# AbbVie-ComputationalGenomics/SAIGEgds

Measured on AMD Instinct MI355X. Metric: variants/sec seqAssocGLMM_SPA at N=430K; achieved HBM GB/s vs roofline, higher is better.
Workload: dtype f64

## Files before the change

saigegds_amd/csrc/kern_score3.h:

```cpp
#pragma once
#include <type_traits>

#ifndef S3_V4I_DEFINED
#define S3_V4I_DEFINED
typedef int s3_v4i __attribute__((ext_vector_type(4)));
#endif

#include "s3_layout.h"

template <int OFF> __device__ __forceinline__ void s3_ds_read(s3_v4i &dst, uint32_t addr)
{
	asm volatile("ds_read_b128 %0, %1 offset:%2" : "=v"(dst) : "v"(addr), "n"(OFF));
}
template <int N> __device__ __forceinline__ void s3_lgkm_wait(s3_v4i &reg) { asm volatile("s_waitcnt lgkmcnt(%1)" : "+v"(reg) : "n"(N)); }
__device__ __forceinline__ void s3_tie(s3_v4i &reg) { asm volatile("" : "+v"(reg)); }
#define S3_DS_READ(dst, addr, off) s3_ds_read<(off)>(dst, addr)
#define S3_LGKM_WAIT(n, reg) s3_lgkm_wait<(n)>(reg)
#define S3_TIE(reg) s3_tie(reg)

template <int I, int N, typename F>
__device__ __forceinline__ void s3_static_for(F &&f)
{
	if constexpr (I < N) { f(std::integral_constant<int, I>()); s3_static_for<I + 1, N>(f); }
}

#ifndef S3_AUX_ROWS
#define S3_AUX_ROWS 2
#endif
#define S3_WAITCNT_VM(n) __builtin_amdgcn_s_waitcnt(((n) & 0xF) | (((n) >> 4) << 14) | (0x7 << 4) | (0xF << 8))

template <int OP>
__device__ __forceinline__ void s3_unpack_op(uint32_t w, uint32_t &w4, s3_v4i &val, s3_v4i &b1)
{
	if constexpr (OP == 0) w4 = w >> 4;
	else if constexpr (OP == 1) val[0] = (int)(w & 0x03030303u);
	else if constexpr (OP == 2) val[1] = (int)(w & 0x0C0C0C0Cu);
	else if constexpr (OP == 3) val[2] = (int)(w4 & 0x03030303u);
	else if constexpr (OP == 4) val[3] = (int)(w4 & 0x0C0C0C0Cu);
	else if constexpr (OP == 5) b1[0] = (int)(w & 0x02020202u);
	else if constexpr (OP == 6) b1[1] = (int)(w & 0x08080808u);
	else if constexpr (OP == 7) b1[2] = (int)(w4 & 0x02020202u);
	else if constexpr (OP == 8) b1[3] = (int)(w4 & 0x08080808u);
}
#define S3_UNPACK3_OPS 15
template <int OP>
__device__ __forceinline__ void s3_unpack3_op(uint32_t w, uint32_t &w4, uint32_t &t, uint32_t &t4, s3_v4i &val, s3_v4i &b1, s3_v4i &mis)
{
	if constexpr (OP < 9) s3_unpack_op<OP>(w, w4, val, b1);
	else if constexpr (OP == 9) t = w >> 1;
	else if constexpr (OP == 10) t4 = w4 >> 1;
	else if constexpr (OP == 11) mis[0] = (int)(w & t & 0x01010101u);
	else if constexpr (OP == 12) mis[1] = (int)(w & t & 0x04040404u);
	else if constexpr (OP == 13) mis[2] = (int)(w4 & t4 & 0x01010101u);
	else if constexpr (OP == 14) mis[3] = (int)(w4 & t4 & 0x04040404u);
}

template <int NBF, int NAF, int NC, int NLA, int NLB, int DA, int DB, int ABL = 0, int NCB = 1, int NBUF_ = 2, int RM = 0, bool MISS = false>
__global__ void __launch_bounds__(64 * (NC + NLA + NLB), (NC + NLA + NLB + 3) / 4)
score3_kernel(const uint8_t *__restrict__ A, const uint8_t *__restrict__ Fl, S3Plan pl, int *__restrict__ out, unsigned long long *__restrict__ stamps)
{
#if __HIP_DEVICE_COMPILE__
	static_assert(NC % NCB == 0 && NCB >= 1 && NCB <= 4, "consumer waves = variant groups x column groups");
	constexpr int NCV = NC / NCB;
	constexpr int NBWMAX = (NBF + NCB - 1) / NCB;
	constexpr int NCOL = 16 * NBF;
	constexpr int TILE_BYTES = 16 * NCOL * 16;
	constexpr int NPB = TILE_BYTES / 1024;
	constexpr int NPA = NCV * NAF;
	constexpr int RA = DA + 1, RB = DB + 1;
	constexpr int SLOT_A = (RM == 1 ? 2 : 1) * NPA * 1024;
	static_assert(DA >= 1 && DB >= 1, "at least one tile ahead");
	extern __shared__ __attribute__((aligned(16))) uint8_t s3_smem[];

	const int tid = threadIdx.x, lane = tid & 63, wid = tid >> 6;
	const int x = blockIdx.x & 7, y = blockIdx.x >> 3;
	const int g = x % pl.ng, i = y * (8 / pl.ng) + x / pl.ng;
	const int nk = pl.rf + (i < pl.rem * pl.f ? 1 : 0);
	const int T0 = 2 * (int)((long long)g * (pl.ntile / 2) / pl.ng), T1 = 2 * (int)((long long)(g + 1) * (pl.ntile / 2) / pl.ng);
	unsigned long long st0 = 0, sr0 = 0;
	if (ABL & 16) { st0 = __builtin_amdgcn_s_memtime(); sr0 = __builtin_amdgcn_s_memrealtime(); }

	struct Pos { int k, t, t1, vtile, id; };
	auto pos_set = [&](Pos &p, int k) {
		p.k = k;
		if (k >= nk) return;
		if (k < pl.rf) { p.vtile = k * pl.wpg + i; p.t = T0; p.t1 = T1; p.id = g * pl.ipg + p.vtile; }
		else {
			const int q = i % pl.f, vv = i / pl.f, len = T1 - T0;
			p.vtile = pl.rf * pl.wpg + vv;
			p.t = T0 + 2 * (q * (len / 2) / pl.f); p.t1 = T0 + 2 * ((q + 1) * (len / 2) / pl.f);
			p.id = g * pl.ipg + pl.rf * pl.wpg + i;
		}
	};
	auto pos_next = [&](Pos &p) { if (++p.t >= p.t1) pos_set(p, p.k + 1); };
	Pos pc;
	pos_set(pc, 0);

	if (wid >= NC) {
		const bool rows = wid < NC + NLA;
		const int l = __builtin_amdgcn_readfirstlane(rows ? wid - NC : wid - NC - NLA);
		const int voff = (rows ? s3_dma_lane(lane) : lane) * 16;
		const unsigned rm_bpv = (unsigned)pl.bpv;
		Pos pa = pc;
		int sl = 0;
		int ahead = 0;
		if (rows && RM == 1) {
			constexpr int PLO = NPA / NLA, NHI = NPA % NLA;
			static_assert(2 * (PLO + 1) * (DA > 1 ? DA - 1 : 1) < 64, "vmcnt range");
			const int li = lane >> 3, lj = lane & 7;
			const int rlast = pl.nrow - 1 - 16 * (pl.nfrag - 1);
			unsigned vo[2], vol[2];
#pragma unroll
			for (int h = 0; h < 2; h++) {
				const unsigned c = (unsigned)(lj ^ ((li >> 1) | (h << 2)));
				vo[h] = (unsigned)(8 * h + li) * rm_bpv + c * 16u;
				vol[h] = (unsigned)min(8 * h + li, rlast) * rm_bpv + c * 16u;
			}
			auto issue = [&]() {
				const size_t f0 = (size_t)pa.vtile * pl.fpw;
				const __amdgpu_buffer_rsrc_t rsA = __builtin_amdgcn_make_buffer_rsrc((void *)(A + f0 * 16 * (size_t)pl.bpv), 0, 0xFFFFFFFFu, 0x00020000);
				const int lastf = pl.nfrag - 1 - (int)f0;
#pragma unroll
				for (int j = 0; j <= PLO; j++) {
					const int p = l + j * NLA;
					if (p >= NPA || (ABL & 2)) break;
					const int pp = min(p, lastf);
					const int so = (int)((unsigned)pp * 16u * rm_bpv + (unsigned)(pa.t >> 1) * 128u);
#pragma unroll
					for (int h = 0; h < 2; h++)
						__builtin_amdgcn_raw_ptr_buffer_load_lds(rsA, (__attribute__((address_space(3))) void *)(s3_smem + RB * TILE_BYTES + sl * SLOT_A + (2 * p + h) * 1024),
							16, (int)(pp == lastf ? vol[h] : vo[h]), so, 0, S3_AUX_ROWS);
				}
				sl = sl + 1 == RA ? 0 : sl + 1;
				pos_next(pa); pos_next(pa);
			};
#pragma unroll
			for (int d = 0; d < DA; d++) if (pa.k < nk) { issue(); ahead++; }
			while (pc.k < nk) {
				if (ahead == DA && DA > 1) { if (l < NHI) S3_WAITCNT_VM(2 * (PLO + 1) * (DA - 1)); else S3_WAITCNT_VM(2 * PLO * (DA - 1)); }
				else S3_WAITCNT_VM(0);
				__builtin_amdgcn_s_barrier();
				ahead--;
				if (pa.k < nk) { issue(); ahead++; }
				pos_next(pc);
				__builtin_amdgcn_s_barrier();
				pos_next(pc);
			}
		} else if (rows) {
			constexpr int PLO = NPA / NLA, NHI = NPA % NLA;
			static_assert((PLO + 1) * (DA - 1) < 64, "vmcnt range");
			auto issue = [&]() {
				const size_t f0 = (size_t)pa.vtile * pl.fpw;
				const __amdgpu_buffer_rsrc_t rsA = __builtin_amdgcn_make_buffer_rsrc(
					(void *)(A + (RM ? f0 * 16 * (size_t)pl.bpv : f0 * pl.ntile * 1024)), 0, 0xFFFFFFFFu, 0x00020000);
				const int lastf = pl.nfrag - 1 - (int)f0;
#pragma unroll
				for (int j = 0; j <= PLO; j++) {
					const int p = l + j * NLA;
					if (p >= NPA || (ABL & 2)) break;
					if constexpr (RM == 1) {
					} else if constexpr (RM == 2) {
						const int pp = min(p, lastf);
						__builtin_amdgcn_raw_ptr_buffer_load_lds(rsA, (__attribute__((address_space(3))) void *)(s3_smem + RB * TILE_BYTES + sl * SLOT_A + p * 1024),
							16, (int)((unsigned)(lane >> 3) * rm_bpv + (unsigned)(lane & 7) * 16u),
							(int)(((unsigned)pp * 16u + (unsigned)(pa.t & 1) * 8u) * rm_bpv + (unsigned)(pa.t >> 1) * 128u), 0, 0);
					} else
					__builtin_amdgcn_raw_ptr_buffer_load_lds(rsA, (__attribute__((address_space(3))) void *)(s3_smem + RB * TILE_BYTES + sl * SLOT_A + p * 1024),
						16, voff, (min(p, lastf) * pl.ntile + pa.t) * 1024, 0, 0);
				}
				sl = sl + 1 == RA ? 0 : sl + 1;
				pos_next(pa);
			};
#pragma unroll
			for (int d = 0; d < DA; d++) if (pa.k < nk) { issue(); ahead++; }
			while (pc.k < nk) {
				if (ahead == DA && DA > 1) { if (l < NHI) S3_WAITCNT_VM((PLO + 1) * (DA - 1)); else S3_WAITCNT_VM(PLO * (DA - 1)); }
				else S3_WAITCNT_VM(0);
				__builtin_amdgcn_s_barrier();
				ahead--;
				if (pa.k < nk) { issue(); ahead++; }
				pos_next(pc);
			}
		} else {
			constexpr int PLO = NPB / NLB, NHI = NPB % NLB;
			static_assert((PLO + 1) * (DB - 1) < 64, "vmcnt range");
			const __amdgpu_buffer_rsrc_t rsB = __builtin_amdgcn_make_buffer_rsrc((void *)Fl, 0, 0xFFFFFFFFu, 0x00020000);
			auto issue = [&]() {
#pragma unroll
				for (int j = 0; j <= PLO; j++) {
					const int b = l + j * NLB;
					if (b >= NPB || (ABL & 4)) break;
					__builtin_amdgcn_raw_ptr_buffer_load_lds(rsB, (__attribute__((address_space(3))) void *)(s3_smem + sl * TILE_BYTES + b * 1024),
						16, voff, pa.t * TILE_BYTES + b * 1024, 0, 0);
				}
				sl = sl + 1 == RB ? 0 : sl + 1;
				pos_next(pa);
			};
#pragma unroll
			for (int d = 0; d < DB; d++) if (pa.k < nk) { issue(); ahead++; }
			while (pc.k < nk) {
				if (ahead == DB && DB > 1) { if (l < NHI) S3_WAITCNT_VM((PLO + 1) * (DB - 1)); else S3_WAITCNT_VM(PLO * (DB - 1)); }
				else S3_WAITCNT_VM(0);
				__builtin_amdgcn_s_barrier();
				ahead--;
				if (pa.k < nk) { issue(); ahead++; }
				pos_next(pc);
			}
		}
		return;
	}

	const int r = lane & 15, kg = lane >> 4;
	const int vg = __builtin_amdgcn_readfirstlane(wid / NCB), cgr = __builtin_amdgcn_readfirstlane(wid % NCB);
	const uint32_t smem_lds = (uint32_t)(uintptr_t)(__attribute__((address_space(3))) uint8_t *)s3_smem;
	const uint32_t ring_lds = smem_lds + RB * TILE_BYTES + vg * (NAF * 1024) + lane * 16;
	const int rm_sig = ((r & 7) >> 1) | ((r >> 3) << 2);
	const uint32_t ring_rm = smem_lds + RB * TILE_BYTES + vg * (NAF * 2048) + (uint32_t)(r >> 3) * 1024u + (uint32_t)(r & 7) * 128u;
	const uint32_t ring_rm0 = ring_rm + (uint32_t)(kg ^ rm_sig) * 16u, ring_rm1 = ring_rm + (uint32_t)((4 + kg) ^ rm_sig) * 16u;

	auto consume = [&](auto CG) {
		constexpr int cg = decltype(CG)::value;
		constexpr int B0 = cg * NBWMAX;
		constexpr int NBW = (NBF - B0 < NBWMAX) ? NBF - B0 : NBWMAX;
		constexpr bool HASB1 = B0 + NBW == NBF;
		static_assert(NBW >= 1, "empty column group");
		const uint32_t bt_lds = smem_lds + (4 * kg * NCOL + r) * 16 + B0 * 256;

		s3_v4i acc[NAF][NBW];
#pragma unroll
		for (int f = 0; f < NAF; f++)
#pragma unroll
			for (int b = 0; b < NBW; b++) acc[f][b] = (s3_v4i){0, 0, 0, 0};

		constexpr int BCH = NBUF_ > 2 ? 1 : NCB > 1 ? (NBW <= 2 ? NBW : 2) : (NBF <= 4 ? NBF : (NBF >= 9 ? 2 : (NBF % 3 == 0 ? 3 : 4)));
		constexpr int NBUF = NBUF_;
		constexpr bool PIPE = NCB == 1 && NBF <= 8;
		constexpr int NCH = (NBW + BCH - 1) / BCH;
		constexpr int NM = NAF * NBW;
		constexpr int NV = HASB1 ? 4 * NAF : 0, NW = 5 * NAF;
		constexpr int BLV = HASB1 ? NBW - 2 : NBW - 1;
		constexpr int MB = HASB1 ? ((!PIPE && NBW >= 3) ? (NBW - 2) * NAF : (NBW - 1) * NAF) : 0;
		static_assert(!HASB1 || NBW >= 2 || NCB == 1, "a column group of the b1 fragment alone has no slot for its unpack");

		int sa = 0, sb = 0;
		int par = 0;
		while (pc.k < nk) {
			__builtin_amdgcn_sched_barrier(0);
			__builtin_amdgcn_s_barrier();
			__builtin_amdgcn_sched_barrier(0);
			const uint32_t a_addr = (RM == 1 ? (par ? ring_rm1 : ring_rm0) : ring_lds) + (uint32_t)(sa * SLOT_A);
			constexpr int AFS = RM == 1 ? 2048 : 1024;
			const uint32_t b_addr = bt_lds + (uint32_t)(sb * TILE_BYTES);
			s3_v4i aw[NAF];
			s3_static_for<0, NAF>([&](auto F) { constexpr int f = decltype(F)::value; S3_DS_READ(aw[f], a_addr, f * AFS); });
			s3_v4i bf[NBUF][BCH];
			auto read_chunk = [&](auto CI) {
				constexpr int ci = decltype(CI)::value, u = ci / NCH, b0 = (ci % NCH) * BCH;
				s3_static_for<0, BCH>([&](auto J) {
					constexpr int j = decltype(J)::value;
					if constexpr (b0 + j < NBW) {
						if (ABL & 8) bf[ci % NBUF][j] = (s3_v4i){u, j, r, sa};
						else S3_DS_READ(bf[ci % NBUF][j], b_addr, u * NCOL * 16 + (b0 + j) * 256);
					}
				});
			};
			constexpr int nread_last = NBW - (NCH - 1) * BCH;
			auto nreads = [](int c0, int c1) constexpr { int n = 0; for (int c = c0; c < c1 && c < 4 * NCH; c++) n += (c % NCH == NCH - 1) ? nread_last : BCH; return n; };
			s3_static_for<0, NBUF - 1>([&](auto C) { if constexpr (decltype(C)::value < 4 * NCH) read_chunk(C); });
			if (!(ABL & 8)) { S3_LGKM_WAIT(nreads(0, NBUF - 1), aw[0]); } else { S3_LGKM_WAIT(0, aw[0]); }
#pragma unroll
			for (int f = 1; f < NAF; f++) S3_TIE(aw[f]);
			s3_v4i val[PIPE ? 2 : 1][NAF], b1[NAF];
			uint32_t w4[PIPE ? 2 : 1][NAF];
			if (!(ABL & 1)) {
				s3_static_for<0, (PIPE ? NW : 5)>([&](auto O) {
					constexpr int o = decltype(O)::value, f = o / 5, op = o % 5;
					s3_unpack_op<op>((uint32_t)aw[f][0], w4[0][f], val[0][f], b1[f]);
				});
			}
			__builtin_amdgcn_sched_barrier(0);
			constexpr bool FM = !PIPE && BCH == 2 && nread_last == 2;
			constexpr int M0 = (NCH - 1) * BCH * NAF;
			s3_static_for<0, 4>([&](auto U) {
				constexpr int u = decltype(U)::value;
				constexpr int vb = PIPE ? (u & 1) : 0, vn = PIPE ? ((u + 1) & 1) : 0;
				s3_static_for<0, NM>([&](auto MI) {
					constexpr int m = decltype(MI)::value;
					constexpr bool fm = FM && m >= M0;
					constexpr int b = fm ? (NCH - 1) * BCH + (m - M0) % 2 : m / NAF, f = fm ? (m - M0) / 2 : m % NAF;
					constexpr int ch = b / BCH, ci = u * NCH + ch, j = b % BCH;
					if constexpr (m == ch * BCH * NAF) {
						if constexpr (ci + NBUF - 1 < 4 * NCH) read_chunk(std::integral_constant<int, ci + NBUF - 1>());
						constexpr int inflight = (ABL & 8) ? 0 : nreads(ci + 1, ci + NBUF);
						constexpr int nb = (ch == NCH - 1) ? nread_last : BCH;
						S3_LGKM_WAIT(inflight, bf[ci % NBUF][0]);
#pragma unroll
						for (int jj = 1; jj < nb; jj++) S3_TIE(bf[ci % NBUF][jj]);
					}
					if (ABL & 1) { if (f == 0) acc[0][b][1] ^= bf[ci % NBUF][j][0] ^ aw[b % NAF][u]; }
					else if (HASB1 && b == NBW - 1) acc[f][b] = __builtin_amdgcn_mfma_i32_16x16x64_i8(b1[f], bf[ci % NBUF][j], acc[f][b], 0, 0, 0);
					else acc[f][b] = __builtin_amdgcn_mfma_i32_16x16x64_i8(val[vb][f], bf[ci % NBUF][j], acc[f][b], 0, 0, 0);
					if (!(ABL & 1)) {
						if constexpr (!PIPE && u == 0 && b == 0 && f + 1 < NAF) {
							s3_static_for<0, 5>([&](auto O) {
								constexpr int op = decltype(O)::value;
								s3_unpack_op<op>((uint32_t)aw[f + 1][0], w4[0][f + 1], val[0][f + 1], b1[f + 1]);
							});
						}
						if constexpr (m < MB) {
							s3_static_for<m * NV / MB, (m + 1) * NV / MB>([&](auto O) {
								constexpr int o = decltype(O)::value, ff = o / 4, op = 5 + o % 4;
								s3_unpack_op<op>((uint32_t)aw[ff][u], w4[vb][ff], val[vb][ff], b1[ff]);
							});
						}
						if constexpr (PIPE && u < 3) {
							s3_static_for<m * NW / NM, (m + 1) * NW / NM>([&](auto O) {
								constexpr int o = decltype(O)::value, ff = o / 5, op = o % 5;
								s3_unpack_op<op>((uint32_t)aw[ff][u + 1], w4[vn][ff], val[vn][ff], b1[ff]);
							});
						}
						if constexpr (!PIPE && u < 3) {
							constexpr int lo = !fm ? ((b == BLV || (BLV < 0 && b == 0)) ? 0 : 5) : (HASB1 ? (j == 0 ? 0 : 2) : (j == 1 ? 0 : 5));
							constexpr int hi = !fm ? 5 : (HASB1 && j == 0 ? 2 : 5);
							s3_static_for<lo, hi>([&](auto O) {
								constexpr int op = decltype(O)::value;
								s3_unpack_op<op>((uint32_t)aw[f][u + 1], w4[0][f], val[0][f], b1[f]);
							});
						}
					}
					__builtin_amdgcn_sched_barrier(0);
				});
			});
			if (pc.t + 1 == pc.t1) {
				int *dst = out + ((size_t)pc.id * NC + wid) * (NAF * NBWMAX * 256) + lane;
#pragma unroll
				for (int f = 0; f < NAF; f++)
#pragma unroll
					for (int b = 0; b < NBW; b++)
#pragma unroll
						for (int reg = 0; reg < 4; reg++) {
							dst[((f * NBWMAX + b) * 4 + reg) * 64] = acc[f][b][reg];
							acc[f][b][reg] = 0;
						}
			}
			pos_next(pc);
			if (RM != 1 || par) sa = sa + 1 == RA ? 0 : sa + 1;
			sb = sb + 1 == RB ? 0 : sb + 1;
			par ^= 1;
		}
	};
	auto consume3 = [&]() {
		static_assert(!MISS || NCB == 1, "the three-plane form has one column group");
		constexpr int NBUF = NBUF_;
		constexpr int NBV = NBF - 1;
		constexpr int NVF = 2 * NBV + 1;
		constexpr int NM = NAF * NVF;
		constexpr int NOPT = S3_UNPACK3_OPS * NAF;
		constexpr int BCH = NBF <= 4 ? NBF : 2, NCH = (NBF + BCH - 1) / BCH;
		const uint32_t bt_lds = smem_lds + (4 * kg * NCOL + r) * 16;
		s3_v4i acc[NAF][NBF], accm[NAF][NBV > 0 ? NBV : 1];
#pragma unroll
		for (int f = 0; f < NAF; f++) {
#pragma unroll
			for (int b = 0; b < NBF; b++) acc[f][b] = (s3_v4i){0, 0, 0, 0};
#pragma unroll
			for (int b = 0; b < NBV; b++) accm[f][b] = (s3_v4i){0, 0, 0, 0};
		}
		int sa = 0, sb = 0, par = 0;
		while (pc.k < nk) {
			__builtin_amdgcn_sched_barrier(0);
			__builtin_amdgcn_s_barrier();
			__builtin_amdgcn_sched_barrier(0);
			const uint32_t a_addr = (RM == 1 ? (par ? ring_rm1 : ring_rm0) : ring_lds) + (uint32_t)(sa * SLOT_A);
			constexpr int AFS = RM == 1 ? 2048 : 1024;
			const uint32_t b_addr = bt_lds + (uint32_t)(sb * TILE_BYTES);
			s3_v4i aw[NAF];
			s3_static_for<0, NAF>([&](auto F) { constexpr int f = decltype(F)::value; S3_DS_READ(aw[f], a_addr, f * AFS); });
			s3_v4i bf[NBUF][BCH];
			auto read_chunk = [&](auto CI) {
				constexpr int ci = decltype(CI)::value, u = ci / NCH, b0 = (ci % NCH) * BCH;
				s3_static_for<0, BCH>([&](auto J) {
					constexpr int j = decltype(J)::value;
					if constexpr (b0 + j < NBF) S3_DS_READ(bf[ci % NBUF][j], b_addr, u * NCOL * 16 + (b0 + j) * 256);
				});
			};
			constexpr int nread_last = NBF - (NCH - 1) * BCH;
			auto nreads = [](int c0, int c1) constexpr { int n = 0; for (int c = c0; c < c1 && c < 4 * NCH; c++) n += (c % NCH == NCH - 1) ? nread_last : BCH; return n; };
			s3_static_for<0, NBUF - 1>([&](auto C) { if constexpr (decltype(C)::value < 4 * NCH) read_chunk(C); });
			S3_LGKM_WAIT(nreads(0, NBUF - 1), aw[0]);
#pragma unroll
			for (int f = 1; f < NAF; f++) S3_TIE(aw[f]);
			s3_v4i val[2][NAF], b1[2][NAF], mis[2][NAF];
			uint32_t w4[NAF], tt[NAF], m4[NAF];
			s3_static_for<0, NOPT>([&](auto O) {
				constexpr int o = decltype(O)::value, f = o / S3_UNPACK3_OPS, op = o % S3_UNPACK3_OPS;
				s3_unpack3_op<op>((uint32_t)aw[f][0], w4[f], tt[f], m4[f], val[0][f], b1[0][f], mis[0][f]);
			});
			__builtin_amdgcn_sched_barrier(0);
			s3_static_for<0, 4>([&](auto U) {
				constexpr int u = decltype(U)::value, vb = u & 1, vn = (u + 1) & 1;
				s3_static_for<0, NM>([&](auto MI) {
					constexpr int m = decltype(MI)::value, vf = m / NAF, f = m % NAF;
					constexpr int b = vf < 2 * NBV ? vf / 2 : NBV;
					constexpr int plane = vf < 2 * NBV ? (vf & 1) : 2;
					constexpr int ch = b / BCH, ci = u * NCH + ch, j = b % BCH;
					if constexpr (f == 0 && plane != 1 && b % BCH == 0) {
						if constexpr (ci + NBUF - 1 < 4 * NCH) read_chunk(std::integral_constant<int, ci + NBUF - 1>());
						constexpr int inflight = nreads(ci + 1, ci + NBUF);
						constexpr int nb = (ch == NCH - 1) ? nread_last : BCH;
						S3_LGKM_WAIT(inflight, bf[ci % NBUF][0]);
#pragma unroll
						for (int jj = 1; jj < nb; jj++) S3_TIE(bf[ci % NBUF][jj]);
					}
					if constexpr (plane == 0) acc[f][b] = __builtin_amdgcn_mfma_i32_16x16x64_i8(val[vb][f], bf[ci % NBUF][j], acc[f][b], 0, 0, 0);
					else if constexpr (plane == 1) accm[f][b] = __builtin_amdgcn_mfma_i32_16x16x64_i8(mis[vb][f], bf[ci % NBUF][j], accm[f][b], 0, 0, 0);
					else acc[f][b] = __builtin_amdgcn_mfma_i32_16x16x64_i8(b1[vb][f], bf[ci % NBUF][j], acc[f][b], 0, 0, 0);
					if constexpr (u < 3) {
						s3_static_for<m * NOPT / NM, (m + 1) * NOPT / NM>([&](auto O) {
							constexpr int o = decltype(O)::value, ff = o / S3_UNPACK3_OPS, op = o % S3_UNPACK3_OPS;
							s3_unpack3_op<op>((uint32_t)aw[ff][u + 1], w4[ff], tt[ff], m4[ff], val[vn][ff], b1[vn][ff], mis[vn][ff]);
						});
					}
					__builtin_amdgcn_sched_barrier(0);
				});
			});
			if (pc.t + 1 == pc.t1) {
				int *dst = out + ((size_t)pc.id * NC + wid) * (NAF * NVF * 256) + lane;
#pragma unroll
				for (int f = 0; f < NAF; f++) {
#pragma unroll
					for (int b = 0; b < NBF; b++)
#pragma unroll
						for (int reg = 0; reg < 4; reg++) { dst[((f * NVF + b) * 4 + reg) * 64] = acc[f][b][reg]; acc[f][b][reg] = 0; }
#pragma unroll
					for (int b = 0; b < NBV; b++)
#pragma unroll
						for (int reg = 0; reg < 4; reg++) { dst[((f * NVF + NBF + b) * 4 + reg) * 64] = accm[f][b][reg]; accm[f][b][reg] = 0; }
				}
			}
			pos_next(pc);
			if (RM != 1 || par) sa = sa + 1 == RA ? 0 : sa + 1;
			sb = sb + 1 == RB ? 0 : sb + 1;
			par ^= 1;
		}
	};
	if constexpr (MISS) consume3();
	else if constexpr (NCB == 1) consume(std::integral_constant<int, 0>());
	else s3_static_for<0, NCB>([&](auto CG) { if (cgr == decltype(CG)::value) consume(CG); });
	if ((ABL & 16) && tid == 0) {
		stamps[2 * blockIdx.x] = __builtin_amdgcn_s_memtime() - st0;
		stamps[2 * blockIdx.x + 1] = __builtin_amdgcn_s_memrealtime() - sr0;
	}
#endif
}

#define S3_FOR_EACH_NBF(X) \
	X(2, 4, 8, 3, 1, 1, 2) X(3, 4, 8, 3, 1, 1, 1) X(4, 4, 8, 3, 1, 1, 1) X(5, 3, 8, 3, 1, 1, 2) X(6, 3, 8, 3, 1, 1, 1) \
	X(7, 4, 4, 2, 2, 2, 1) X(8, 4, 4, 2, 2, 2, 1) X(9, 4, 4, 2, 2, 1, 1) X(10, 4, 4, 2, 2, 1, 1) X(11, 4, 4, 2, 2, 1, 1) \
	X(12, 3, 4, 2, 2, 1, 1) X(13, 3, 4, 2, 2, 1, 1) X(14, 2, 4, 2, 2, 2, 1) X(15, 2, 4, 2, 2, 1, 1) X(16, 2, 4, 2, 2, 1, 1)
#define S3_FOR_EACH_NBF_MISS(X) \
	X(2, 4, 8, 3, 1, 1, 2) X(3, 3, 8, 3, 1, 1, 2) X(4, 2, 8, 3, 1, 2, 2) X(5, 2, 8, 3, 1, 2, 2) X(6, 3, 4, 2, 2, 2, 1) \
	X(7, 2, 4, 2, 2, 2, 1) X(8, 2, 4, 2, 2, 2, 1) X(9, 2, 4, 2, 2, 2, 1) X(10, 2, 4, 2, 2, 2, 1) X(11, 1, 4, 2, 2, 2, 1) \
	X(12, 1, 4, 2, 2, 2, 1) X(13, 1, 4, 2, 2, 2, 1) X(14, 1, 4, 2, 2, 2, 1) X(15, 1, 4, 2, 2, 2, 1) X(16, 1, 4, 2, 2, 2, 1)
static inline size_t s3_lds_bytes(int NBF, int NAF, int NC, int DA, int DB) { return ((size_t)(DB + 1) * 4 * NBF + (size_t)(DA + 1) * 2 * NC * NAF) * 1024; }

#ifndef S3_KERNEL_ONLY
#include "kern_lists.h"

__device__ __forceinline__ unsigned long long s3_block_excl(unsigned long long x, unsigned long long *sh)
{
	const int tid = threadIdx.x;
	sh[tid] = x;
	__syncthreads();
	for (int o = 1; o < 1024; o <<= 1) {
		const unsigned long long y = tid >= o ? sh[tid - o] : 0;
		__syncthreads();
		sh[tid] += y;
		__syncthreads();
	}
	const unsigned long long incl = sh[tid];
	__syncthreads();
	return incl - x;
}

__global__ void __launch_bounds__(256)
s3_ingest_clist_count_kernel(int M, int N, int lim, int *__restrict__ nzv ,
	const int *__restrict__ n2v, const int *__restrict__ n3, uint8_t *__restrict__ corient)
{
	const int v = blockIdx.x * 256 + threadIdx.x;
	if (v >= M) return;
	const int nz = nzv[v], n2 = n2v[v], m3 = n3[v];
	const long long AC = (long long)(nz - n2 - m3) + 2ll * n2;
	const bool minus = (double)AC / (2.0 * (double)(N - m3)) > 0.5;
	const int nnz = minus ? N - n2 : nz;
	const int orient = (N - m3 > 0 && nnz <= lim) ? (minus ? 2 : 1) : 0;
	corient[v] = (uint8_t)orient;
	nzv[v] = orient ? nnz : 0;
}

__global__ void __launch_bounds__(1024)
s3_ingest_clist_kernel(int M, unsigned cidx_cap, const int *__restrict__ cn, unsigned *__restrict__ cptr, uint8_t *__restrict__ corient)
{
	__shared__ unsigned long long sh[1024];
	const int tid = threadIdx.x, per = (M + 1023) / 1024, v0 = tid * per, v1 = min(M, v0 + per);
	unsigned long long mine = 0;
	for (int v = v0; v < v1; v++) mine += (unsigned long long)cn[v];
	unsigned long long base = s3_block_excl(mine, sh);
	for (int v = v0; v < v1; v++) {
		const int n = cn[v];
		const bool fits = base + (unsigned long long)n <= (unsigned long long)cidx_cap;
		cptr[v] = (unsigned)min(base, (unsigned long long)cidx_cap);
		if (!fits) corient[v] = 0;
		else base += (unsigned long long)n;
	}
	if (tid == 1023) cptr[M] = (unsigned)min(base, (unsigned long long)cidx_cap);
}

template <int PP>
__global__ void __launch_bounds__(256, PP <= 16 ? 8 : 7)
s3_t3_kernel(int M, int P, const long long *__restrict__ Q, S3Lists L, long long *__restrict__ part)
{
	constexpr int TPW = 64 / PP;
	constexpr int NB = 1;
	const int lane = threadIdx.x & 63, wid = threadIdx.x >> 6;
	const int g = blockIdx.x % L.nr, chunk = blockIdx.x / L.nr;
	const unsigned *__restrict__ idx = L.idx;
	const int c = lane % PP, tk = lane / PP;
	const int v = (chunk * 4 + wid) * TPW + tk;
	unsigned e0 = 0, e1 = 0;
	if (v < M) { e0 = L.lstart[(size_t)g * L.ld + v]; e1 = e0 + (unsigned)max(0, L.lcnt[(size_t)g * L.ld + v]); }
	long long hi = 0, lo = 0;
	const int gbase = lane - c;
	for (unsigned e = e0; __any(e < e1); e += NB * PP) {
		unsigned mine[NB];
#pragma unroll
		for (int k = 0; k < NB; k++) mine[k] = (e + k * PP + c < e1) ? idx[e + k * PP + c] : 0xFFFFFFFFu;
		constexpr int UN = PP <= 16 ? 8 : 4;
		constexpr int UNR = PP <= 16 ? 2 : 1;
#pragma unroll
		for (int k = 0; k < NB; k++)
#pragma unroll UNR
			for (int j0 = 0; j0 < PP; j0 += UN) {
				long long q[UN];
#pragma unroll
				for (int j = 0; j < UN; j++) {
					const unsigned s = (unsigned)__shfl((int)mine[k], gbase + j0 + j, 64);
					q[j] = (s != 0xFFFFFFFFu && c < P) ? Q[(size_t)s * P + c] : 0;
				}
#pragma unroll
				for (int j = 0; j < UN; j++) { hi += q[j] >> 32; lo += q[j] & 0xFFFFFFFFll; }
			}
	}
	if (v < M && c < P) {
		long long *o = part + (((size_t)g * M + v) * P + c) * 2;
		o[0] = hi; o[1] = lo;
	}
}

__global__ void __launch_bounds__(256)
s3_reduce_kernel(S3Plan pl, int M, int NCW, int NAF, int NBF, int NCB, const int *__restrict__ slabs, int *__restrict__ accbuf, int stride,
	int *__restrict__ counters, int *__restrict__ cursors)
{
	if (blockIdx.x == 0 && blockIdx.y == 0 && threadIdx.x < 32) {
		if (threadIdx.x < 24) counters[threadIdx.x] = 0;
		if (threadIdx.x < 8 && cursors) cursors[threadIdx.x] = 0;
	}
	const int NBW = (NBF + NCB - 1) / NCB;
	const int e = (blockIdx.x * 256 + threadIdx.x) * 4, per = NCW * NAF * NBW * 256, vtile = blockIdx.y;
	if (e >= per) return;
	const int lane = e & 63, reg = (e >> 6) & 3, fb = e >> 8;
	const int bw = fb % NBW, wf = fb / NBW;
	const int wave = wf / NAF, f = wf - wave * NAF;
	const int b = (wave % NCB) * NBW + bw;
	if (b >= NBF) return;
	const int v = (vtile * pl.fpw + (wave / NCB) * NAF + f) * 16 + (lane >> 4) * 4 + reg;
	if (v >= M) return;
	s3_v4i sum = (s3_v4i){0, 0, 0, 0};
	for (int g = 0; g < pl.ng; g++) {
		int first, count;
		s3_items_of(pl, vtile, g, first, count);
		for (int id = first; id < first + count; id++) sum += *reinterpret_cast<const s3_v4i *>(slabs + (size_t)id * per + e);
	}
	*reinterpret_cast<s3_v4i *>(accbuf + (size_t)v * stride + b * 16 + (lane & 15)) = sum;
}

__host__ __device__ constexpr int s3e_vb(int K) { return K <= 8 ? 256 : 128; }
template <int K>
__global__ void __launch_bounds__(256)
score3_epilogue(int M, DevModel md, MfEpi ep, const int *__restrict__ accbuf, int acc_stride, int miss_off,
	const long long *__restrict__ t3part , int nr,
	const int *__restrict__ lcnt , size_t ld, int *__restrict__ ovf_list,
	SpaRec *__restrict__ recs, int *__restrict__ counters, int btop, int *__restrict__ fb_series, int *__restrict__ fb_exact,
	double *__restrict__ out8, uint8_t *__restrict__ valid, double guard_tol, int dbg = 0)
{
	constexpr int P = 2 * K + 2, CW = P - 1;
	constexpr int S3E_VB = s3e_vb(K);
	__shared__ double s_acc[S3E_VB][P | 1];
	__shared__ double s_imp[S3E_VB];
	__shared__ int s_n[S3E_VB][4];
	__shared__ long long s_ftot[P][2];
	__shared__ int s_col[P][3];
	const int tid = threadIdx.x, j0 = blockIdx.x * S3E_VB;
	const int N = md.N;
	if (dbg & 1) {
		if (tid == 0)
#pragma unroll
			for (int c = 0; c < P; c++) {
				s_col[c][0] = ep.ccol[c]; s_col[c][1] = ep.climb[c]; s_col[c][2] = ep.escale[c];
				s_ftot[c][0] = ep.ftot_hi[c]; s_ftot[c][1] = ep.ftot_lo[c];
			}
	} else
	for (int c = tid; c < P; c += S3E_VB) {
		s_col[c][0] = ep.ccol[c]; s_col[c][1] = ep.climb[c]; s_col[c][2] = ep.escale[c];
		s_ftot[c][0] = ep.ftot_hi[c]; s_ftot[c][1] = ep.ftot_lo[c];
	}
	{
		const int j = j0 + tid;
		const int *a0 = accbuf + (size_t)min(j, M - 1) * acc_stride;
		int n3 = 0;
		bool over = false;
		if (miss_off) n3 = a0[miss_off + ep.col_ones] / 4;
		else {
			for (int g0 = 0; g0 < nr; g0 += 8) {
				int cn[8];
#pragma unroll
				for (int u = 0; u < 8; u++) cn[u] = lcnt[(size_t)min(g0 + u, nr - 1) * ld + min(j, M - 1)];
#pragma unroll
				for (int u = 0; u < 8; u++) if (g0 + u < nr) { over |= cn[u] < 0; n3 += cn[u] < 0 ? 0 : cn[u]; }
			}
		}
		if (j >= M) n3 = 0;
		{
			const int tot = wave_total_i(n3);
			if ((tid & 63) == 0 && tot >= 64) atomicAdd(&counters[22], tot >> 6);
		}
		int state = 0, n1 = 0, n2 = 0;
		double imp = 0;
		if (dbg & 8) over = false;
		if (j < M) {
			if (over) ovf_list[atomicAdd(&counters[23], 1)] = j;
			else {
				const long long AC = (long long)(a0[ep.col_ones] / 4) - 3ll * n3;
				n2 = a0[ep.col_b1 + ep.climb[CW]] / 8 - n3;
				n1 = (int)(AC - 2ll * n2);
				const VarHead h = make_head(md, (double)AC, N - n3);
				if (!h.pass) { nan_row(out8 + (size_t)j * 8); valid[j] = 0; }
				else { state = h.minus ? 2 : 1; imp = 2 * h.AF; }
			}
		}
		s_n[tid][0] = n1; s_n[tid][1] = n2; s_n[tid][2] = n3; s_n[tid][3] = state;
		s_imp[tid] = imp;
	}
	__syncthreads();
	for (int task = tid; task < S3E_VB * P; task += S3E_VB) {
		const int vl = task / P, c = task - vl * P, j = j0 + vl;
		const int state = s_n[vl][3];
		if (!state) continue;
		const int cc = s_col[c][0], nl = s_col[c][1];
		if (nl == 0) { s_acc[vl][c] = 0; continue; }
		const int *a0 = accbuf + (size_t)j * acc_stride;
		const bool minus = state == 2;
		const double imp = s_imp[vl];
		int lv[MF_NLIMB], lm[MF_NLIMB], lb[MF_NLIMB];
#pragma unroll
		for (int l = 0; l < MF_NLIMB; l++) lv[l] = a0[cc + min(l, nl - 1)];
		HiLo T3 = hl(0, 0);
		if (miss_off) {
#pragma unroll
			for (int l = 0; l < MF_NLIMB; l++) lm[l] = a0[miss_off + cc + min(l, nl - 1)];
		} else if (!(dbg & 2)) {
			const long long *p = t3part + ((size_t)j * P + c) * 2;
			const size_t gs = (size_t)M * P * 2;
			for (int g0 = 0; g0 < nr; g0 += 8) {
				long long ph[8], pl[8];
#pragma unroll
				for (int u = 0; u < 8; u++) { const long long *q = p + (size_t)min(g0 + u, nr - 1) * gs; ph[u] = q[0]; pl[u] = q[1]; }
#pragma unroll
				for (int u = 0; u < 8; u++) if (g0 + u < nr) { T3.hi += ph[u]; T3.lo += pl[u]; }
			}
		}
		if (c == CW) {
#pragma unroll
			for (int l = 0; l < MF_NLIMB; l++) lb[l] = a0[ep.col_b1 + min(l, nl - 1)];
		}
		auto limbs = [&](const int (&x)[MF_NLIMB]) -> HiLo {
			long long lo = 0, hi = 0;
#pragma unroll
			for (int l = 3; l >= 0; l--) lo = lo * 256 + (l < nl ? x[l] : 0);
#pragma unroll
			for (int l = MF_NLIMB - 1; l >= 4; l--) hi = hi * 256 + (l < nl ? x[l] : 0);
			return hl(hi, lo);
		};
		const HiLo V = limbs(lv);
		if (miss_off) T3 = limbs(lm);
		const HiLo W = hl_axpy(-3, T3, V);
		const double t3d = hl_to_double(T3);
		double r;
		if (c != CW) {
			double sm;
			if (!minus) sm = hl_to_double(W) + imp * t3d;
			else sm = hl_to_double(hl(2 * s_ftot[c][0] - W.hi, 2 * s_ftot[c][1] - W.lo)) - imp * t3d;
			r = ldexp(sm, -s_col[c][2]);
		} else {
			const HiLo B2 = limbs(lb);
			const HiLo H2 = hl(B2.hi / 2 - T3.hi, B2.lo / 2 - T3.lo);
			double w;
			if (!minus) {
				w = hl_to_double(hl_axpy(2, H2, W)) + imp * imp * t3d;
			} else {
				const HiLo S1 = hl_axpy(-2, H2, W);
				const HiLo R = hl(s_ftot[CW][0] - S1.hi - H2.hi - T3.hi, s_ftot[CW][1] - S1.lo - H2.lo - T3.lo);
				w = hl_to_double(hl_axpy(4, R, S1)) + (2 - imp) * (2 - imp) * t3d;
			}
			r = ldexp(w, -s_col[CW][2]);
		}
		s_acc[vl][c] = r;
	}
	__syncthreads();
	if (dbg & 4) return;
	const int j = j0 + tid;
	if (j >= M || !s_n[tid][3]) return;
	const int n1 = s_n[tid][0], n2 = s_n[tid][1], n3 = s_n[tid][2];
	const long long AC = (long long)n1 + 2ll * n2;
	const VarHead h = make_head(md, (double)AC, N - n3);
	const double imp = 2 * h.AF;
	double *o = out8 + (size_t)j * 8;
	double acc[P];
#pragma unroll
	for (int c = 0; c < P; c++) acc[c] = s_acc[tid][c];
	if (ep.derive_c) {
#pragma unroll
		for (int x = 0; x < K; x++) {
			double cx = 0;
#pragma unroll
			for (int y = 0; y < K; y++) cx = fma(ep.XVXi[x * K + y], acc[K + y], cx);
			acc[x] = cx;
		}
	}
	{
		const double g2 = (double)n1 + 4.0 * n2 + (h.minus ? (2 - imp) * (2 - imp) : imp * imp) * n3;
		const double spread = 8.0 * sqrt(fmax(g2, 1.0));
		double dcol[P];
#pragma unroll
		for (int c = 0; c < P; c++) dcol[c] = (ep.climb[c] && !(md.quant && c == CW)) ? spread * ldexp(1.0, -ep.escale[c]) : 0.0;
		double sat[K];
#pragma unroll
		for (int y = 0; y < K; y++) {
			double t = 0;
#pragma unroll
			for (int x = 0; x < K; x++) t = fma(md.S_a[x], ep.XVXi[x * K + y], t);
			sat[y] = t;
		}
		double dquad = 0, dec = 0, dS = dcol[2 * K], quad = 0, ec = 0, sac = 0;
#pragma unroll
		for (int a = 0; a < K; a++) {
			double t = 0;
#pragma unroll
			for (int b = 0; b < K; b++) t = fma(md.XVX[a * K + b], acc[b], t);
			quad = fma(t, acc[a], quad);
			dquad += 2 * dcol[a] * fabs(t - acc[K + a]);
			ec = fma(acc[K + a], acc[a], ec);
			dec += dcol[K + a] * fabs(acc[a]);
			sac = fma(md.S_a[a], acc[a], sac);
			dS += ep.derive_c ? fabs(sat[a]) * dcol[K + a] : fabs(md.S_a[a]) * dcol[a];
		}
		const double var2 = quad + acc[CW] - 2 * ec, S = acc[2 * K] - sac;
		const double dvar = dquad + 2 * dec + dcol[CW];
		const double sd = sqrt(md.r * fmax(var2, 0.0) * (md.quant ? 1.0 / fmax(h.mac, 1.0) : 1.0)) * (md.quant ? md.tau0 * sqrt(fmax(h.mac, 1.0)) : 1.0);
		const double z = fabs(S) / sd;
		const double dz = dS / sd + 0.5 * z * dvar / var2;
		if (!(dz * fmax(1.0, z) <= guard_tol)) {
			ovf_list[atomicAdd(&counters[23], 1)] = j;
			atomicAdd(&counters[21], 1);
			return;
		}
	}
	double cbuf[KMAX], pn, Ssc, v2sc;
	valid[j] = 1;
	if (score_epilogue<(P - 2) / 2>(md, h, acc, o, cbuf, &pn, &Ssc, &v2sc)) {
		spa_push<K>(md, recs, counters, btop, fb_series, fb_exact, j, h.minus, h.minus ? (2 * h.Num - h.AC) : h.AC,
			h.minus ? (N - n2) : (n1 + n2 + n3), h.lut, pn, Ssc, v2sc, cbuf);
	}
	{
		const unsigned long long act = __ballot(true);
		if (__builtin_amdgcn_mbcnt_hi((uint32_t)(act >> 32), __builtin_amdgcn_mbcnt_lo((uint32_t)act, 0u)) == 0u) atomicAdd(&counters[1], (int)__popcll(act));
	}
}
#endif
```

Baseline: 16.66 million.

## Single-buffer unpack planes via compile-time MFMA/unpack schedule for NBF=4 missing-data kernel

For the three-plane (missing-aware) consumer with NBF=4 and at least three A fragments, the unpacked value/bit/missing planes are kept in one register set instead of double-buffered. A constexpr schedule reorders the MFMAs and places each unpack op between its earliest safe slot and its deadline, and a static_assert checks that every op lands before the MFMA that reads it. The B fragments are read in a permuted chunk order to match. The lower register use lets the NBF=4 MISS configuration move from 2 to 3 A fragments with shallower A buffering, trading register pressure for more reuse of each B tile, at the cost of tighter instruction ordering.

```diff
diff --git a/saigegds_amd/csrc/kern_score3.h b/saigegds_amd/csrc/kern_score3.h
--- a/saigegds_amd/csrc/kern_score3.h
+++ b/saigegds_amd/csrc/kern_score3.h
@@ -54,6 +54,55 @@
 	else if constexpr (OP == 13) mis[2] = (int)(w4 & t4 & 0x01010101u);
 	else if constexpr (OP == 14) mis[3] = (int)(w4 & t4 & 0x04040404u);
 }
+
+template <int NAF>
+struct s3_one {
+	static constexpr int NM = 7 * NAF, NOPT = S3_UNPACK3_OPS * NAF, DL = 2, NK = 3 * NOPT;
+	static constexpr int piece_of(int m) { return m < NAF ? m : m < 3 * NAF ? (m - NAF) / 2 : (m - 3 * NAF) / 4; }
+	static constexpr int frag_of(int m) { return m < NAF ? 3 : m < 3 * NAF ? 0 : 1 + ((m - 3 * NAF) & 3) / 2; }
+	static constexpr int plane_of(int m) { return m < NAF ? 2 : m < 3 * NAF ? (m - NAF) & 1 : (m - 3 * NAF) & 1; }
+	static constexpr int chunk_of(int m) { return m < 3 * NAF ? 0 : 1; }
+	static constexpr int slot_of(int m) { return m < NAF ? 0 : m < 3 * NAF ? 1 : ((m - 3 * NAF) & 3) / 2; }
+	static constexpr int frag(int ch, int j) { return ch == 0 ? (j == 0 ? 3 : 0) : 1 + j; }
+	static constexpr bool enters(int m) { return m == 0 || m == 3 * NAF; }
+	static constexpr int piece(int i) { return i < 7 * NAF ? i / 7 : (i - 7 * NAF) / 8; }
+	static constexpr int op(int i)
+	{
+		const int head[7] = {0, 9, 10, 5, 6, 7, 8}, tail[8] = {1, 2, 3, 4, 11, 12, 13, 14};
+		return i < 7 * NAF ? head[i % 7] : tail[(i - 7 * NAF) % 8];
+	}
+	static constexpr int earliest(int d, int i)
+	{
+		const int base = NM * (d - 1);
+		if (i < 7 * NAF) return base + (i % 7 >= 3 ? i / 7 : 0);
+		const int q = i - 7 * NAF;
+		return base + 3 * NAF + 4 * (q / 8) + (q % 8 < 4 ? 2 : 3);
+	}
+	static constexpr int deadline(int d, int i)
+	{
+		const int base = NM * d;
+		if (i < 7 * NAF) return i % 7 >= 3 ? base + i / 7 : 1 << 30;
+		const int q = i - 7 * NAF;
+		return base + NAF + 2 * (q / 8) + (q % 8 < 4 ? 0 : 1);
+	}
+	static constexpr int slot(int k)
+	{
+		int s = 0;
+		for (int j = 0; j <= k; j++) {
+			const int d = 1 + j / NOPT, i = j % NOPT, t = NM * (d - 1) + i * NM / NOPT + DL, e = earliest(d, i);
+			s = s > t ? s : t;
+			s = s > e ? s : e;
+		}
+		return s;
+	}
+	static constexpr int first(int g) { int k = 0; while (k < NK && slot(k) < g) k++; return k; }
+	static constexpr bool ok()
+	{
+		for (int k = 0; k < NK; k++)
+			if (slot(k) >= deadline(1 + k / NOPT, k % NOPT) || slot(k) >= 4 * NM) return false;
+		return true;
+	}
+};
 
 template <int NBF, int NAF, int NC, int NLA, int NLB, int DA, int DB, int ABL = 0, int NCB = 1, int NBUF_ = 2, int RM = 0, bool MISS = false>
 __global__ void __launch_bounds__(64 * (NC + NLA + NLB), (NC + NLA + NLB + 3) / 4)
@@ -356,7 +405,11 @@
 		constexpr int NVF = 2 * NBV + 1;
 		constexpr int NM = NAF * NVF;
 		constexpr int NOPT = S3_UNPACK3_OPS * NAF;
-		constexpr int BCH = NBF <= 4 ? NBF : 2, NCH = (NBF + BCH - 1) / BCH;
+		constexpr bool ONE = NBF == 4 && NAF >= 3;
+		using S1 = s3_one<NAF>;
+		static_assert(!ONE || S1::ok(), "an unpack operation of the one-set schedule lands behind the MFMA that needs it");
+		constexpr int BCH = ONE ? 2 : NBF <= 4 ? NBF : 2, NCH = (NBF + BCH - 1) / BCH;
+		constexpr int NPS = ONE ? 1 : 2;
 		const uint32_t bt_lds = smem_lds + (4 * kg * NCOL + r) * 16;
 		s3_v4i acc[NAF][NBF], accm[NAF][NBV > 0 ? NBV : 1];
 #pragma unroll
@@ -381,7 +434,8 @@
 				constexpr int ci = decltype(CI)::value, u = ci / NCH, b0 = (ci % NCH) * BCH;
 				s3_static_for<0, BCH>([&](auto J) {
 					constexpr int j = decltype(J)::value;
-					if constexpr (b0 + j < NBF) S3_DS_READ(bf[ci % NBUF][j], b_addr, u * NCOL * 16 + (b0 + j) * 256);
+					constexpr int b = ONE ? S1::frag(ci % NCH, j) : b0 + j;
+					if constexpr (b0 + j < NBF) S3_DS_READ(bf[ci % NBUF][j], b_addr, u * NCOL * 16 + b * 256);
 				});
 			};
 			constexpr int nread_last = NBF - (NCH - 1) * BCH;
@@ -390,7 +444,7 @@
 			S3_LGKM_WAIT(nreads(0, NBUF - 1), aw[0]);
 #pragma unroll
 			for (int f = 1; f < NAF; f++) S3_TIE(aw[f]);
-			s3_v4i val[2][NAF], b1[2][NAF], mis[2][NAF];
+			s3_v4i val[NPS][NAF], b1[NPS][NAF], mis[NPS][NAF];
 			uint32_t w4[NAF], tt[NAF], m4[NAF];
 			s3_static_for<0, NOPT>([&](auto O) {
 				constexpr int o = decltype(O)::value, f = o / S3_UNPACK3_OPS, op = o % S3_UNPACK3_OPS;
@@ -398,13 +452,14 @@
 			});
 			__builtin_amdgcn_sched_barrier(0);
 			s3_static_for<0, 4>([&](auto U) {
-				constexpr int u = decltype(U)::value, vb = u & 1, vn = (u + 1) & 1;
+				constexpr int u = decltype(U)::value, vb = ONE ? 0 : u & 1, vn = ONE ? 0 : (u + 1) & 1;
 				s3_static_for<0, NM>([&](auto MI) {
-					constexpr int m = decltype(MI)::value, vf = m / NAF, f = m % NAF;
-					constexpr int b = vf < 2 * NBV ? vf / 2 : NBV;
-					constexpr int plane = vf < 2 * NBV ? (vf & 1) : 2;
-					constexpr int ch = b / BCH, ci = u * NCH + ch, j = b % BCH;
-					if constexpr (f == 0 && plane != 1 && b % BCH == 0) {
+					constexpr int m = decltype(MI)::value, vf = m / NAF;
+					constexpr int f = ONE ? S1::piece_of(m) : m % NAF;
+					constexpr int b = ONE ? S1::frag_of(m) : vf < 2 * NBV ? vf / 2 : NBV;
+					constexpr int plane = ONE ? S1::plane_of(m) : vf < 2 * NBV ? (vf & 1) : 2;
+					constexpr int ch = ONE ? S1::chunk_of(m) : b / BCH, ci = u * NCH + ch, j = ONE ? S1::slot_of(m) : b % BCH;
+					if constexpr (ONE ? S1::enters(m) : f == 0 && plane != 1 && b % BCH == 0) {
 						if constexpr (ci + NBUF - 1 < 4 * NCH) read_chunk(std::integral_constant<int, ci + NBUF - 1>());
 						constexpr int inflight = nreads(ci + 1, ci + NBUF);
 						constexpr int nb = (ch == NCH - 1) ? nread_last : BCH;
@@ -415,7 +470,13 @@
 					if constexpr (plane == 0) acc[f][b] = __builtin_amdgcn_mfma_i32_16x16x64_i8(val[vb][f], bf[ci % NBUF][j], acc[f][b], 0, 0, 0);
 					else if constexpr (plane == 1) accm[f][b] = __builtin_amdgcn_mfma_i32_16x16x64_i8(mis[vb][f], bf[ci % NBUF][j], accm[f][b], 0, 0, 0);
 					else acc[f][b] = __builtin_amdgcn_mfma_i32_16x16x64_i8(b1[vb][f], bf[ci % NBUF][j], acc[f][b], 0, 0, 0);
-					if constexpr (u < 3) {
+					if constexpr (ONE) {
+						constexpr int g = u * NM + m;
+						s3_static_for<S1::first(g), S1::first(g + 1)>([&](auto K) {
+							constexpr int k = decltype(K)::value, d = 1 + k / NOPT, i = k % NOPT, ff = S1::piece(i), op = S1::op(i);
+							s3_unpack3_op<op>((uint32_t)aw[ff][d], w4[ff], tt[ff], m4[ff], val[0][ff], b1[0][ff], mis[0][ff]);
+						});
+					} else if constexpr (u < 3) {
 						s3_static_for<m * NOPT / NM, (m + 1) * NOPT / NM>([&](auto O) {
 							constexpr int o = decltype(O)::value, ff = o / S3_UNPACK3_OPS, op = o % S3_UNPACK3_OPS;
 							s3_unpack3_op<op>((uint32_t)aw[ff][u + 1], w4[ff], tt[ff], m4[ff], val[vn][ff], b1[vn][ff], mis[vn][ff]);
@@ -459,7 +520,7 @@
 	X(7, 4, 4, 2, 2, 2, 1) X(8, 4, 4, 2, 2, 2, 1) X(9, 4, 4, 2, 2, 1, 1) X(10, 4, 4, 2, 2, 1, 1) X(11, 4, 4, 2, 2, 1, 1) \
 	X(12, 3, 4, 2, 2, 1, 1) X(13, 3, 4, 2, 2, 1, 1) X(14, 2, 4, 2, 2, 2, 1) X(15, 2, 4, 2, 2, 1, 1) X(16, 2, 4, 2, 2, 1, 1)
 #define S3_FOR_EACH_NBF_MISS(X) \
-	X(2, 4, 8, 3, 1, 1, 2) X(3, 3, 8, 3, 1, 1, 2) X(4, 2, 8, 3, 1, 2, 2) X(5, 2, 8, 3, 1, 2, 2) X(6, 3, 4, 2, 2, 2, 1) \
+	X(2, 4, 8, 3, 1, 1, 2) X(3, 3, 8, 3, 1, 1, 2) X(4, 3, 8, 3, 1, 1, 2) X(5, 2, 8, 3, 1, 2, 2) X(6, 3, 4, 2, 2, 2, 1) \
 	X(7, 2, 4, 2, 2, 2, 1) X(8, 2, 4, 2, 2, 2, 1) X(9, 2, 4, 2, 2, 2, 1) X(10, 2, 4, 2, 2, 2, 1) X(11, 1, 4, 2, 2, 2, 1) \
 	X(12, 1, 4, 2, 2, 2, 1) X(13, 1, 4, 2, 2, 2, 1) X(14, 1, 4, 2, 2, 2, 1) X(15, 1, 4, 2, 2, 2, 1) X(16, 1, 4, 2, 2, 2, 1)
 static inline size_t s3_lds_bytes(int NBF, int NAF, int NC, int DA, int DB) { return ((size_t)(DB + 1) * 4 * NBF + (size_t)(DA + 1) * 2 * NC * NAF) * 1024; }
```

Measured after the change: 18.11 million (median of 6 runs). +8.7%, better.
